# baggepinnen/LPVSpectral.jl

Hardware: AMD Instinct MI355X
Metric: signals/sec, ls_sparse_spectral_lpv group lasso N=2^20 Nf=512 Nv=8 (2000 ADMM iters; iters/sec in admm_iters_per_sec) (higher is better)
Workload: dtype f64

## Files before the change

lpvspectral.jl_amd/csrc/admm_one_launch.hip:

```cpp
#include "lpvs_internal.h"
#include "admm_device.h"
#include "admm_host.h"
#include "tile_order.h"

#include <algorithm>
#include <map>
#include <mutex>
#include <tuple>
#include <vector>
#include <cmath>
#include <cstdlib>
#include <string>
#include <type_traits>

namespace lpvs {

enum { FI_FIRST = 0, FI_MID = 1, FI_LAST = 2 };
typedef void (*FiKernel)(AdmmParams, const unsigned char *, const unsigned char *, int, int, long long, int, int, int, size_t, int);
static FiKernel fi_kernel(int mode, bool small, bool batch, bool nt, bool pa, bool f32);

__device__ __forceinline__ double wave_max(double v) {
#pragma unroll
    for (int o = 32; o > 0; o >>= 1) v = fmax(v, __shfl_xor(v, o, 64));
    return v;
// ... 41 lines not shown
    const int64_t r = (int64_t)blockIdx.x * 4 + wave;
    if (r >= n) return;
    const double2 *m2 = reinterpret_cast<const double2 *>(M + ((int64_t)blockIdx.y * np + r) * np);
    double acc = 0;
    for (int64_t j = lane; j < np / 2; j += 64) { const double2 m = m2[j]; acc += fabs(m.x) + fabs(m.y); }
    acc = wave_sum(acc);
    if (lane == 0) atomicMax(out + 2 * blockIdx.y, (unsigned long long)__double_as_longlong(acc));
}
__global__ void __launch_bounds__(256)
fi_state_kernel(AdmmParams p, int nblk, long long base, int with_consts) {
    const int sg = blockIdx.x, nprob = gridDim.x;
    const FiBufs f = fi_views(p.fi, (int64_t)nprob * p.np, nprob * nblk, nprob);
    const int64_t voff = (int64_t)sg * p.np;
    __shared__ double sh[3][4];
    double mx = 0, mr = 0, mu_ = 0;
    int bad = 0;
    for (int64_t e = threadIdx.x; e < p.np; e += 256) {
        const double a = p.xb[voff + e], b = p.rhs[voff + e], c = p.u[voff + e];
        mx = fmax(mx, fabs(a)); mr = fmax(mr, fabs(b)); mu_ = fmax(mu_, fabs(c));
        bad |= !(fabs(b) < 0x1p1000) || !(fabs(c) < 0x1p1000);
    }
    mx = wave_max(mx); mr = wave_max(mr); mu_ = wave_max(mu_);
    if ((threadIdx.x & 63) == 0) { sh[0][threadIdx.x >> 6] = mx; sh[1][threadIdx.x >> 6] = mr; sh[2][threadIdx.x >> 6] = mu_; }
    __syncthreads();
    mx = fmax(fmax(sh[0][0], sh[0][1]), fmax(sh[0][2], sh[0][3]));
    mr = fmax(fmax(sh[1][0], sh[1][1]), fmax(sh[1][2], sh[1][3]));
    mu_ = fmax(fmax(sh[2][0], sh[2][1]), fmax(sh[2][2], sh[2][3]));
    if (__syncthreads_or(bad)) { mr = __longlong_as_double(0x7ff0000000000000ll); mu_ = mr; }
    const int p1 = (int)((base + 1) & 1), p2 = (int)(base & 1);
    const int nbt = nprob * nblk, boff = sg * nblk;
    for (int b = threadIdx.x; b < nblk; b += 256) {
        f.rec[p1 * nbt + boff + b] = make_double2(mr, mu_);
        f.rec[p2 * nbt + boff + b] = make_double2(0.0, p.mu * mr);
        f.bn[boff + b] = 0.0; f.bn[nbt + boff + b] = 0.0;
    }
    if (threadIdx.x == 0) {
        if (with_consts) f.consts[2 * sg + 1] = mx;
        f.qbuf[sg] = 0.0; f.qbuf[nprob + sg] = 0.0;
    }
}

__device__ __forceinline__ void fi_fixed_product(const FixRaw &fr, const double *sI, const double *sJ, int wave, int lane, double (&v)[8], double (&tc)[8]) {
    const int c = lane & 15, gq = lane >> 4;
    double rj[8];
#pragma unroll
    for (int k = 0; k < 4; ++k) { rj[k] = sJ[4 * c + k]; rj[4 + k] = sJ[64 + 4 * c + k]; }
#pragma unroll
    for (int k = 0; k < 8; ++k) tc[k] = 0.0;
    const float stv[8] = {fr.st[0].x, fr.st[0].y, fr.st[0].z, fr.st[0].w, fr.st[1].x, fr.st[1].y, fr.st[1].z, fr.st[1].w};
    const unsigned int nw[8] = {fr.nq[0].x, fr.nq[0].y, fr.nq[0].z, fr.nq[0].w, fr.nq[1].x, fr.nq[1].y, fr.nq[1].z, fr.nq[1].w};
    double ri = (double)stv[0] * sI[wave * 32 + gq];
#pragma unroll
    for (int rg = 0; rg < 8; ++rg) {
        const double step = (double)stv[rg];
        const double ri_next = rg + 1 < 8 ? (double)stv[rg + 1] * sI[wave * 32 + 4 * (rg + 1) + gq] : 0.0;
        const int hh[8] = {fr.ha[rg].x, fr.ha[rg].y, fr.ha[rg].z, fr.ha[rg].w, fr.hb[rg].x, fr.hb[rg].y, fr.hb[rg].z, fr.hb[rg].w};
        double a0 = 0.0, a1 = 0.0;
#pragma unroll
        for (int k = 0; k < 8; k += 2) {
            const double m0 = fix_decode((unsigned int)hh[k], (nw[rg] >> (4 * k)) & 15u);
            const double m1 = fix_decode((unsigned int)hh[k + 1], (nw[rg] >> (4 * k + 4)) & 15u);
            tc[k] = opaque(fma(m0, ri, tc[k]));
            tc[k + 1] = opaque(fma(m1, ri, tc[k + 1]));
            a0 = fma(m0, rj[k], a0);
            a1 = fma(m1, rj[k + 1], a1);
        }
        v[rg] = step * (a0 + a1);
        ri = ri_next;
        __builtin_amdgcn_sched_barrier(0);
    }
}


#if defined(LPVS_TIMELINE) && LPVS_TIMELINE < 3
__device__ unsigned long long *g_lpvs_tl = nullptr;
extern "C" int32_t lpvs_debug_set_timeline(unsigned long long *dev_buf) {
    return hipMemcpyToSymbol(HIP_SYMBOL(g_lpvs_tl), &dev_buf, sizeof(dev_buf)) == hipSuccess ? LPVS_OK : LPVS_EDEVICE;
}
#define LPVS_TL_STAMP(k) do { if ((LPVS_TIMELINE >= 2 || (k) == 5) && tl_on && threadIdx.x == 0) tl_rec[k] = __builtin_amdgcn_s_memrealtime(); } while (0)
#else
#define LPVS_TL_STAMP(k) do { } while (0)
#endif

template <int MODE, int NK, bool BATCH, bool NT, bool PA, bool F32, bool NIBR = false>
__device__ __forceinline__ void
fi_one_tile_body(const AdmmParams &p, const unsigned char *__restrict__ Mp, const unsigned char *__restrict__ types, int ntiles, int nblk, long long g, int aslot,
                 int uslot , int commit_prev, size_t mp_stride) {
    constexpr bool prefetch_all = PA;
#if defined(LPVS_TIMELINE) && LPVS_TIMELINE < 3
    const bool tl_on = MODE == FI_MID && !BATCH && !F32 && g_lpvs_tl != nullptr;
    unsigned long long *tl_rec = tl_on ? g_lpvs_tl + ((size_t)(g & 1) * (size_t)ntiles + blockIdx.x) * 8 : nullptr;
    if (tl_on && threadIdx.x == 0) {
        tl_rec[0] = (unsigned long long)g; tl_rec[1] = __builtin_amdgcn_s_memrealtime();
        tl_rec[7] = __builtin_amdgcn_s_getreg((32 - 1) << 11 | 0 << 6 | 4);
    }
#endif
    __shared__ double sI[TS], sJ[TS], sT[4][TS], sq[2 * TS], red[3][4];
    const int sg = BATCH ? (int)blockIdx.y : 0, nprob = BATCH ? (int)gridDim.y : 1;
    const int64_t voff = (int64_t)sg * p.np;
    const int boff = sg * nblk, nbt = nprob * nblk;
    const FiBufs f = fi_views(p.fi, (int64_t)nprob * p.np, nbt, nprob);
    Mp += (size_t)sg * mp_stride; types += (size_t)sg * (size_t)ntiles;
    const int lane = threadIdx.x & 63, wave = threadIdx.x >> 6;
    const int bx = (MODE == FI_LAST || BATCH) ? (int)blockIdx.x : tile_order_index((int)blockIdx.x, nblk, p.tile_order & (int)(g & 1));
    int I, J;
    if (MODE == FI_LAST || bx < nblk) { I = J = bx; }
    else {
        const int k = bx - nblk;
        I = (int)((1.0 + sqrt(1.0 + 8.0 * (double)k)) * 0.5);
        while (I * (I - 1) / 2 > k) --I;
        while ((I + 1) * I / 2 <= k) ++I;
        J = k - I * (I - 1) / 2;
    }
    const int t = I * (I + 1) / 2 + J;
#if defined(LPVS_TIMELINE) && LPVS_TIMELINE < 3
    if (tl_on && threadIdx.x == 0) tl_rec[6] = __builtin_amdgcn_s_getreg((4 - 1) << 11 | 0 << 6 | 20) | (unsigned long long)t << 8;
#endif
    const unsigned char *tile = Mp + (size_t)t * (F32 ? (size_t)TS * TS * 4 : kSplitTileBytes);
    const unsigned char ttype = (MODE == FI_LAST || F32) ? 0 : types[t];
    AdmmStatus *status = p.status + sg;
    const int conv_flag = __builtin_nontemporal_load(&status->converged);
    const int blk = threadIdx.x < TS ? I : J, i = threadIdx.x & (TS - 1);
    const int64_t e = (int64_t)blk * TS + i;
    const bool ok = e < p.n;
    const int pg = (int)(g & 1), pg1 = pg ^ 1;
    double rhs_mem = 0, xbv = 0, uv = 0, qprev = 0;
    long long accp = 0;
    if (MODE == FI_FIRST) rhs_mem = p.rhs[voff + e];
    else {
        accp = f.acc((aslot + 2) % 3)[voff + e];
        xbv = p.xb[voff + e];
        uv = (uslot ? f.ualt : p.u)[voff + e];
        qprev = f.qbuf[pg1 * nprob + sg];
    }
    double bnv[NK];
    double2 recv[NK];
#pragma unroll
    for (int k = 0; k < NK; ++k) {
        const int b = lane + 64 * k < nblk ? lane + 64 * k : nblk - 1;
        bnv[k] = MODE != FI_FIRST ? f.bn[pg * nbt + boff + b] : 0.0;
        recv[k] = MODE != FI_LAST ? f.rec[pg * nbt + boff + b] : make_double2(0.0, 0.0);
    }
    const double Rrow = BATCH ? f.consts[2 * sg] : p.fi_R, xbmax = BATCH ? f.consts[2 * sg + 1] : p.fi_xbmax;
    __builtin_amdgcn_sched_barrier(0);
    FixRaw fr;
    float4 fha[8], fhb[8];
    double diag_pre = 0.0;
    if (MODE != FI_LAST && F32) {
        typedef unsigned int u32x4b __attribute__((ext_vector_type(4)));
        const __amdgpu_buffer_rsrc_t rs = __builtin_amdgcn_make_buffer_rsrc(const_cast<unsigned char *>(tile), 0, TS * TS * 4, 0x00020000);
        const int off_head = ((wave * 32 + (lane >> 4)) * TS + 4 * (lane & 15)) * 4;
#pragma unroll
        for (int rg = 0; rg < 8; ++rg) {
            fha[rg] = __builtin_bit_cast(float4, (u32x4b)__builtin_amdgcn_raw_buffer_load_b128(rs, off_head, rg * (4 * TS * 4), 0));
            fhb[rg] = __builtin_bit_cast(float4, (u32x4b)__builtin_amdgcn_raw_buffer_load_b128(rs, off_head, rg * (4 * TS * 4) + 256, 0));
        }
    }
    if (MODE != FI_LAST && !F32) {
        typedef unsigned int u32x4b __attribute__((ext_vector_type(4)));
        constexpr int aux = NT ? 2 : 0;
        const int tbytes = I != J ? (int)kMixedFixedTileBytes : (prefetch_all ? (int)kMixedFixedTileBytes + TS * 8 : 0);
        const __amdgpu_buffer_rsrc_t rs = __builtin_amdgcn_make_buffer_rsrc(const_cast<unsigned char *>(tile), 0, tbytes, 0x00020000);
        const __amdgpu_buffer_rsrc_t rs_nq = __builtin_amdgcn_make_buffer_rsrc(const_cast<unsigned char *>(tile), 0, p.mp_fix32 ? 0 : tbytes, 0x00020000);
        const int gq_ = lane >> 4, c_ = lane & 15;
        const int off_head = ((wave * 32 + gq_) * TS + 4 * c_) * 4;
        const int off_nq = (int)kFixHeadBytes + (wave * 64 + lane) * 32, off_st = (int)(kFixHeadBytes + kFixNibBytes) + (wave * 4 + gq_) * 32;
        fr.nq[0] = __builtin_bit_cast(uint4, (u32x4b)__builtin_amdgcn_raw_buffer_load_b128(rs_nq, off_nq, 0, aux));
        fr.nq[1] = __builtin_bit_cast(uint4, (u32x4b)__builtin_amdgcn_raw_buffer_load_b128(rs_nq, off_nq, 16, aux));
        fr.st[0] = __builtin_bit_cast(float4, (u32x4b)__builtin_amdgcn_raw_buffer_load_b128(rs, off_st, 0, aux));
        fr.st[1] = __builtin_bit_cast(float4, (u32x4b)__builtin_amdgcn_raw_buffer_load_b128(rs, off_st, 16, aux));
#pragma unroll
        for (int rg = 0; rg < 8; ++rg) {
            fr.ha[rg] = __builtin_bit_cast(int4, (u32x4b)__builtin_amdgcn_raw_buffer_load_b128(rs, off_head, rg * (4 * TS * 4), aux));
            fr.hb[rg] = __builtin_bit_cast(int4, (u32x4b)__builtin_amdgcn_raw_buffer_load_b128(rs, off_head, rg * (4 * TS * 4) + 256, aux));
        }
        if (PA) {
            const int rgo = ((c_ & 8) ? 4 : 0) + ((c_ & 4) ? 2 : 0) + ((c_ & 2) ? 1 : 0);
            typedef unsigned int u32x2b __attribute__((ext_vector_type(2)));
            const u32x2b dw = __builtin_amdgcn_raw_buffer_load_b64(rs, (int)(kFixHeadBytes + kFixNibBytes) + TS * 4 + (wave * 32 + 4 * rgo + gq_) * 8, 0, 0);
            diag_pre = __builtin_bit_cast(double, dw);
        }
    }
    __builtin_amdgcn_sched_barrier(0);
    double mR = 0, mU = 0;
#pragma unroll
    for (int k = 0; k < NK; ++k) { mR = fmax(mR, recv[k].x); mU = fmax(mU, recv[k].y); }
    if (conv_flag) return;
    if (MODE != FI_FIRST && commit_prev && (p.tol > 0.0 || blockIdx.x == 0)) {
        double part = 0.0;
#pragma unroll
        for (int k = 0; k < NK; ++k) part += lane + 64 * k < nblk ? bnv[k] : 0.0;
        const double nxz = sqrt(wave_sum(part));
        const bool conv = nxz < p.tol;
        if (blockIdx.x == 0 && threadIdx.x == 0) commit_iteration(status, nxz, p.tol);
        if (conv) return;
    }
    double rhs_v;
    if (MODE == FI_FIRST) rhs_v = rhs_mem;
    else {
        const double xi = ok ? xbv + (double)accp * qprev : 0.0;
        const double ui = ok ? uv : 0.0;
        const double v = xi + ui;
        double zi = 0.0;
        if (p.prox_kind == LPVS_PROX_L1) {
            zi = prox_l1(v, p.mu * p.prox_param);
        } else if (p.prox_kind == LPVS_PROX_L0) {
            zi = prox_l0(v, sqrt(2.0 * p.mu * p.prox_param));
        } else {
            const int gl = (int)p.group_len;
            sq[threadIdx.x] = v * v;
            __syncthreads();
            const double *grp = sq + (threadIdx.x & TS) + (i / gl) * gl;
            double s2 = 0;
            for (int q = 0; q < gl; ++q) s2 += grp[q];
            zi = group_scale(s2, p.prox_param * p.mu) * v;
        }
        if (!ok) zi = 0.0;
        const DualStep t = dual_step(xi, ui, zi, 0.0, p.mu, ok, true);
        const double d = t.d, un = t.un;
        rhs_v = t.rhs;
        if (I == J) {
            const bool own = threadIdx.x < TS;
            if (own) {
                p.x[voff + e] = xi; p.z[voff + e] = zi;
                (MODE == FI_LAST ? p.u : (uslot ? p.u : f.ualt))[voff + e] = un;
                if (MODE == FI_LAST) p.rhs[voff + e] = rhs_v;
            }
            const double d2 = own && ok ? d * d : 0.0;
            const double inf_ = __longlong_as_double(0x7ff0000000000000ll);
            const double ar = fabs(rhs_v) < inf_ ? fabs(rhs_v) : inf_, au = fabs(un) < inf_ ? fabs(un) : inf_;
            const double w0 = wave_sum(d2), w1 = wave_max(own ? ar : 0.0), w2 = wave_max(own ? au : 0.0);
            if (lane == 0) { red[0][wave] = w0; red[1][wave] = w1; red[2][wave] = w2; }
            __syncthreads();
            if (threadIdx.x == 0) {
                f.bn[pg1 * nbt + boff + I] = red[0][0] + red[0][1];
                f.rec[pg1 * nbt + boff + I] = make_double2(fmax(red[1][0], red[1][1]), fmax(red[2][0], red[2][1]));
            }
        }
    }
    if (MODE == FI_LAST) return;
    LPVS_TL_STAMP(2);
    if (I == J && threadIdx.x < TS) f.acc((aslot + 1) % 3)[voff + e] = 0;
    if (threadIdx.x < TS) sI[i] = rhs_v; else sJ[i] = rhs_v;
    mR = wave_max_nonneg(mR); mU = wave_max_nonneg(mU);
    double B = Rrow * ((xbmax + Rrow * mR + mU) / p.mu) * 1.000001;
    const bool bound_ok = B < 0x1p1000;
    if (!(B > 0x1p-900)) B = 0x1p-900;
    int eb = 0;
    (void)frexp(bound_ok ? B : 1.0, &eb);
    const double quantum = bound_ok ? ldexp(1.0, eb - 62) : __longlong_as_double(0x7ff8000000000000ll), invq = bound_ok ? ldexp(1.0, 62 - eb) : 0.0;
    if (blockIdx.x == 0 && threadIdx.x == 0) f.qbuf[pg * nprob + sg] = quantum;
    __syncthreads();
    LPVS_TL_STAMP(3);
    const int c = lane & 15, gq = lane >> 4;
    double rj[8], tc[8], v[8];
    const double *diag = nullptr;
    if (F32) {
#pragma unroll
        for (int k = 0; k < 4; ++k) { rj[k] = sJ[4 * c + k]; rj[4 + k] = sJ[64 + 4 * c + k]; }
#pragma unroll
        for (int k = 0; k < 8; ++k) tc[k] = 0.0;
#pragma unroll
        for (int rg = 0; rg < 8; ++rg) {
            const double ri = sI[wave * 32 + 4 * rg + gq];
            const float hh[8] = {fha[rg].x, fha[rg].y, fha[rg].z, fha[rg].w, fhb[rg].x, fhb[rg].y, fhb[rg].z, fhb[rg].w};
            double a0 = 0.0, a1 = 0.0;
#pragma unroll
            for (int k = 0; k < 8; k += 2) {
                const double m0 = (double)hh[k], m1 = (double)hh[k + 1];
                tc[k] = opaque(fma(m0, ri, tc[k]));
                tc[k + 1] = opaque(fma(m1, ri, tc[k + 1]));
                a0 = fma(m0, rj[k], a0);
                a1 = fma(m1, rj[k + 1], a1);
            }
            v[rg] = a0 + a1;
            __builtin_amdgcn_sched_barrier(0);
        }
    } else if (PA || ttype != 0) {
        if (!PA && I == J) {
            FixRaw fd;
            fix_load(tile, wave, lane, fd, p.mp_fix32 != 0 ? 1 : 0);
            fi_fixed_product(fd, sI, sJ, wave, lane, v, tc);
        } else fi_fixed_product(fr, sI, sJ, wave, lane, v, tc);
        if (ttype == 2 && !prefetch_all) diag = reinterpret_cast<const double *>(tile + kFixHeadBytes + kFixNibBytes + TS * 4);
    } else {
#pragma unroll
        for (int k = 0; k < 4; ++k) { rj[k] = sJ[4 * c + k]; rj[4 + k] = sJ[64 + 4 * c + k]; }
#pragma unroll
        for (int k = 0; k < 8; ++k) tc[k] = 0.0;
        const float *head = reinterpret_cast<const float *>(tile) + (wave * 32 + gq) * TS + 4 * c;
        const unsigned short *tail = reinterpret_cast<const unsigned short *>(tile + (size_t)TS * TS * 4) + (wave * 32 + gq) * TS + 8 * c;
#pragma unroll
        for (int half = 0; half < 2; ++half) {
            float4 ha[4], hb[4];
            uint4 lq[4];
#pragma unroll
            for (int r4 = 0; r4 < 4; ++r4) {
                const int rg = 4 * half + r4;
                ha[r4] = load16<NT, float4>(head + rg * 4 * TS);
                hb[r4] = load16<NT, float4>(head + rg * 4 * TS + 64);
                lq[r4] = load16<NT, uint4>(tail + rg * 4 * TS);
            }
#pragma unroll
            for (int r4 = 0; r4 < 4; ++r4) {
                const int rg = 4 * half + r4;
                const double ri = sI[wave * 32 + 4 * rg + gq];
                const float hh[8] = {ha[r4].x, ha[r4].y, ha[r4].z, ha[r4].w, hb[r4].x, hb[r4].y, hb[r4].z, hb[r4].w};
                const unsigned int qq[8] = {lq[r4].x & 0xffffu, lq[r4].x >> 16, lq[r4].y & 0xffffu, lq[r4].y >> 16,
                                            lq[r4].z & 0xffffu, lq[r4].z >> 16, lq[r4].w & 0xffffu, lq[r4].w >> 16};
                double a0 = 0.0, a1 = 0.0;
#pragma unroll
                for (int k = 0; k < 8; k += 2) {
                    const double m0 = split_decode(hh[k], qq[k]), m1 = split_decode(hh[k + 1], qq[k + 1]);
                    tc[k] = opaque(fma(m0, ri, tc[k]));
                    tc[k + 1] = opaque(fma(m1, ri, tc[k + 1]));
                    a0 = fma(m0, rj[k], a0);
                    a1 = fma(m1, rj[k + 1], a1);
                }
                v[rg] = a0 + a1;
            }
        }
    }
    LPVS_TL_STAMP(4);
#pragma unroll
    for (int m = 8, cnt = 4; m >= 2; m >>= 1, cnt >>= 1) {
        const bool up = (c & m) != 0;
#pragma unroll
        for (int k = 0; k < cnt; ++k) {
            const double lo_ = opaque(v[k]), hi_ = opaque(v[k + cnt]);
            v[k] = (up ? hi_ : lo_) + __shfl_xor(up ? lo_ : hi_, m, 64);
        }
    }
    v[0] += __shfl_xor(v[0], 1, 64);
    unsigned long long *acc_cur = reinterpret_cast<unsigned long long *>(f.acc(aslot));
    if ((c & 1) == 0) {
        const int rg = ((c & 8) ? 4 : 0) + ((c & 4) ? 2 : 0) + ((c & 2) ? 1 : 0);
        const int row = wave * 32 + 4 * rg + gq;
        const double r1 = diag != nullptr ? fma(diag[row], sI[row], v[0]) : (PA && I == J ? fma(diag_pre, sI[row], v[0]) : v[0]);
        atomicAdd(acc_cur + voff + (int64_t)I * TS + row, (unsigned long long)__double2ll_rn(r1 * invq));
    }
    if (I != J) {
#pragma unroll
        for (int m = 32, cnt = 4; m >= 16; m >>= 1, cnt >>= 1) {
            const bool up = (lane & m) != 0;
#pragma unroll
            for (int k = 0; k < cnt; ++k) {
                const double lo_ = opaque(tc[k]), hi_ = opaque(tc[k + cnt]);
                tc[k] = (up ? hi_ : lo_) + __shfl_xor(up ? lo_ : hi_, m, 64);
            }
        }
        const int col = ((lane & 32) ? 64 : 0) + 4 * c + ((lane & 16) ? 2 : 0);
        sT[wave][col] = tc[0]; sT[wave][col + 1] = tc[1];
        __syncthreads();
        if (threadIdx.x < TS) {
            const double r2 = ((sT[0][threadIdx.x] + sT[1][threadIdx.x]) + sT[2][threadIdx.x]) + sT[3][threadIdx.x];
            atomicAdd(acc_cur + voff + (int64_t)J * TS + threadIdx.x, (unsigned long long)__double2ll_rn(r2 * invq));
        }
    }
    if constexpr (NIBR && !F32) {
        if (ttype != 0) {
            __syncthreads();
            FixRaw fb;
            fix_load(tile, wave, lane, fb, 2);
            double vn[8], tn[8];
            fi_fixed_product(fb, sI, sJ, wave, lane, vn, tn);
            unsigned long long *acc_n = reinterpret_cast<unsigned long long *>(p.nib_acc);
#pragma unroll
            for (int m = 8, cnt = 4; m >= 2; m >>= 1, cnt >>= 1) {
                const bool up = (c & m) != 0;
#pragma unroll
                for (int k = 0; k < cnt; ++k) {
                    const double lo_ = opaque(vn[k]), hi_ = opaque(vn[k + cnt]);
                    vn[k] = (up ? hi_ : lo_) + __shfl_xor(up ? lo_ : hi_, m, 64);
                }
            }
            vn[0] += __shfl_xor(vn[0], 1, 64);
            if ((c & 1) == 0) {
                const int rg = ((c & 8) ? 4 : 0) + ((c & 4) ? 2 : 0) + ((c & 2) ? 1 : 0);
                atomicAdd(acc_n + voff + (int64_t)I * TS + wave * 32 + 4 * rg + gq, (unsigned long long)__double2ll_rn(vn[0] * invq));
            }
            if (I != J) {
#pragma unroll
                for (int m = 32, cnt = 4; m >= 16; m >>= 1, cnt >>= 1) {
                    const bool up = (lane & m) != 0;
#pragma unroll
                    for (int k = 0; k < cnt; ++k) {
                        const double lo_ = opaque(tn[k]), hi_ = opaque(tn[k + cnt]);
                        tn[k] = (up ? hi_ : lo_) + __shfl_xor(up ? lo_ : hi_, m, 64);
                    }
                }
                const int col = ((lane & 32) ? 64 : 0) + 4 * c + ((lane & 16) ? 2 : 0);
                sT[wave][col] = tn[0]; sT[wave][col + 1] = tn[1];
                __syncthreads();
                if (threadIdx.x < TS) {
                    const double r2 = ((sT[0][threadIdx.x] + sT[1][threadIdx.x]) + sT[2][threadIdx.x]) + sT[3][threadIdx.x];
                    atomicAdd(acc_n + voff + (int64_t)J * TS + threadIdx.x, (unsigned long long)__double2ll_rn(r2 * invq));
                }
            }
        }
    }
    LPVS_TL_STAMP(5);
}

template <int MODE, int NK, bool BATCH, bool NT, bool PA, bool F32, bool NIBR = false>
__global__ void __launch_bounds__(256, 3)
admm_iter_mixed_kernel(AdmmParams p, const unsigned char *__restrict__ Mp, const unsigned char *__restrict__ types, int ntiles, int nblk, long long g, int aslot,
                       int uslot, int commit_prev, size_t mp_stride, int ) {
    fi_one_tile_body<MODE, NK, BATCH, NT, PA, F32, NIBR>(p, Mp, types, ntiles, nblk, g, aslot, uslot, commit_prev, mp_stride);
}
__global__ void __launch_bounds__(256)
nib_acc_commit_kernel(long long *__restrict__ acc, const double *__restrict__ quantum, const double *__restrict__ xb_corr, double *__restrict__ xb, int64_t np) {
    const int64_t i = (int64_t)blockIdx.x * 256 + threadIdx.x;
    if (i >= np) return;
    const int64_t e = (int64_t)blockIdx.y * np + i;
    xb[e] = xb_corr[e] + (double)acc[e] * quantum[blockIdx.y];
    acc[e] = 0;
}

__global__ void set_double_kernel(double *dst, double v) { *dst = v; }
int32_t launch_fi_setup(const AdmmParams &p, long long base, bool with_consts, hipStream_t s, double r_known) {
    const int nblk = (int)(p.np / TS), nprob = p.ns;
    const FiBufs f = fi_views(p.fi, (int64_t)nprob * p.np, nprob * nblk, nprob);
    if (with_consts) {
        LPVS_HIP(hipMemsetAsync(f.consts, 0, sizeof(double) * 2 * (size_t)nprob, s));
        if (r_known > 0 && nprob == 1) hipLaunchKernelGGL(set_double_kernel, dim3(1), dim3(1), 0, s, f.consts, r_known);
        else hipLaunchKernelGGL(fi_rowsum_kernel, dim3((unsigned)ceil_div(p.np, 4), (unsigned)nprob), dim3(256), 0, s, p.M, p.np, p.n, reinterpret_cast<unsigned long long *>(f.consts));
    }
    hipLaunchKernelGGL(fi_state_kernel, dim3((unsigned)nprob), dim3(256), 0, s, p, nblk, base, with_consts ? 1 : 0);
    LPVS_HIP(hipGetLastError());
    return LPVS_OK;
}

__global__ void __launch_bounds__(256)
fi_fixup_kernel(AdmmParams p, int nblk, long long base, long long iters) {
    const int sg = blockIdx.y, nprob = gridDim.y;
    const AdmmStatus *status = p.status + sg;
    if (!status->converged) return;
    const long long ic = status->iters - base - 1;
    if (ic < 0 || ic > iters - 2 || ((ic + 1) & 1) == 0) return;
    const FiBufs f = fi_views(p.fi, (int64_t)nprob * p.np, nprob * nblk, nprob);
    const int64_t e = (int64_t)blockIdx.x * 256 + threadIdx.x;
    if (e < p.np) p.u[(int64_t)sg * p.np + e] = f.ualt[(int64_t)sg * p.np + e];
}
__global__ void __launch_bounds__(64)
fi_commit_kernel(AdmmParams p, int nblk, int par) {
    const int sg = blockIdx.x, nprob = gridDim.x;
    AdmmStatus *status = p.status + sg;
    if (status->converged) return;
    const FiBufs f = fi_views(p.fi, (int64_t)nprob * p.np, nprob * nblk, nprob);
    __shared__ double slot;
    const double nxz = pending_norm(f.bn + (int64_t)par * nprob * nblk + (int64_t)sg * nblk, nblk, &slot);
    if (threadIdx.x == 0) commit_iteration(status, nxz, p.tol);
}

int32_t fi_read_consts(const AdmmParams &p, double out[2], hipStream_t s) {
    const FiBufs f = fi_views(p.fi, p.np, (int)(p.np / TS));
    LPVS_HIP(hipMemcpyAsync(out, f.consts, sizeof(double) * 2, hipMemcpyDeviceToHost, s));
    LPVS_HIP(hipStreamSynchronize(s));
    return LPVS_OK;
}

template <int NK, bool BATCH, bool NT, bool PA, bool F32 = false>
static FiKernel fi_kernel_mode(int mode) {
    return mode == FI_FIRST ? admm_iter_mixed_kernel<FI_FIRST, NK, BATCH, NT, PA, F32> : mode == FI_MID ? admm_iter_mixed_kernel<FI_MID, NK, BATCH, NT, PA, F32>
                                                                                                       : admm_iter_mixed_kernel<FI_LAST, NK, BATCH, NT, PA, F32>;
}
static FiKernel fi_kernel(int mode, bool small, bool batch, bool nt, bool pa, bool f32 = false) {
    if (f32) return small ? fi_kernel_mode<1, false, false, true, true>(mode) : fi_kernel_mode<6, false, false, true, true>(mode);
    if (batch) {
        if (nt) return pa ? fi_kernel_mode<1, true, true, true>(mode) : fi_kernel_mode<1, true, true, false>(mode);
        return pa ? fi_kernel_mode<1, true, false, true>(mode) : fi_kernel_mode<1, true, false, false>(mode);
    }
    if (small) return pa ? fi_kernel_mode<1, false, false, true>(mode) : fi_kernel_mode<1, false, false, false>(mode);
    if (nt) return pa ? fi_kernel_mode<6, false, true, true>(mode) : fi_kernel_mode<6, false, true, false>(mode);
    return pa ? fi_kernel_mode<6, false, false, true>(mode) : fi_kernel_mode<6, false, false, false>(mode);
}
bool nib_fused_applies(const AdmmParams &p) {
    const char *e = experiment_env("LPVS_NIB_FUSED");
    return !(e && e[0] == '0') && p.nib_period > 0 && p.nib_acc != nullptr && p.mp_types != nullptr && p.fi_prefetch_all == 0 && fi_applicable(p);
}
template <bool NT, bool PA> static FiKernel fi_kernel_nibr_batch(int mode) {
    return mode == FI_FIRST ? admm_iter_mixed_kernel<FI_FIRST, 1, true, NT, PA, false, true> : admm_iter_mixed_kernel<FI_MID, 1, true, NT, PA, false, true>;
}
static FiKernel fi_kernel_nibr(int mode, bool small, bool nt, bool batch = false, bool pa = false) {
    if (batch) { if (nt) return pa ? fi_kernel_nibr_batch<true, true>(mode) : fi_kernel_nibr_batch<true, false>(mode);
                 return pa ? fi_kernel_nibr_batch<false, true>(mode) : fi_kernel_nibr_batch<false, false>(mode); }
    if (small) return mode == FI_FIRST ? admm_iter_mixed_kernel<FI_FIRST, 1, false, false, false, false, true> : admm_iter_mixed_kernel<FI_MID, 1, false, false, false, false, true>;
    if (nt) return mode == FI_FIRST ? admm_iter_mixed_kernel<FI_FIRST, 6, false, true, false, false, true> : admm_iter_mixed_kernel<FI_MID, 6, false, true, false, false, true>;
    return mode == FI_FIRST ? admm_iter_mixed_kernel<FI_FIRST, 6, false, false, false, false, true> : admm_iter_mixed_kernel<FI_MID, 6, false, false, false, false, true>;
}
int32_t launch_fi_chunk(const AdmmParams &p, int64_t iters, bool batch, size_t mp_stride, bool prefetch_all, hipStream_t s) {
    const int nblk = (int)(p.np / TS), nprob = batch ? p.ns : 1;
    const unsigned ntiles = (unsigned)(nblk * (nblk + 1) / 2);
    const FiBufs f = fi_views(p.fi, (int64_t)nprob * p.np, nprob * nblk, nprob);
    const unsigned char *Mp = reinterpret_cast<const unsigned char *>(p.Mp);
    LPVS_HIP(hipMemsetAsync(f.acc(0), 0, sizeof(long long) * (size_t)p.np * (size_t)nprob, s));
    const long long base = p.fi_base;
    const bool small = nblk <= 64;
    const int nto = option_in_effect(LPVS_OPT_NT_LOADS, p.opt_nt_loads);
    const size_t stream_bytes = batch ? (size_t)ntiles * kSplitTileBytes * (size_t)nprob : (size_t)ntiles * kMixedFixedTileBytes;
    const bool nt = (batch || !small) && !p.mp_f32 && (nto ? nto == LPVS_NT_ON : stream_bytes > ((size_t)240 << 20));
    auto launch = [&](int mode, unsigned grid, long long g, int aslot, int uslot, int commit_prev) {
        hipLaunchKernelGGL(fi_kernel(mode, small, batch, nt, prefetch_all, p.mp_f32 != 0), dim3(grid, (unsigned)nprob), dim3(256), 0, s, p, Mp, p.mp_types, (int)ntiles, nblk, g, aslot, uslot,
                           commit_prev, mp_stride, prefetch_all ? 1 : 0);
    };
    const bool nib = batch ? (p.nib_period > 0 && p.nib_acc != nullptr && p.xb_corr != nullptr && p.mp_types != nullptr) : (!prefetch_all && nib_fused_applies(p));
    auto refresh_due = [&](long long g) { return p.nib_period > 0 && nib_refresh_due(g, p.nib_period, p.nib_ramp); };
    auto launch_step = [&](int mode, long long g, int aslot, int uslot, int commit_prev, const double *u_after) -> int32_t {
        const bool due = refresh_due(g);
        if (due && nib) {
            hipLaunchKernelGGL(fi_kernel_nibr(mode, small, nt, batch, prefetch_all), dim3(ntiles, (unsigned)nprob), dim3(256), 0, s, p, Mp, p.mp_types, (int)ntiles, nblk, g, aslot, uslot, commit_prev,
                               mp_stride, prefetch_all ? 1 : 0);
            hipLaunchKernelGGL(nib_acc_commit_kernel, dim3((unsigned)ceil_div(p.np, 256), (unsigned)nprob), dim3(256), 0, s, p.nib_acc, (const double *)(f.qbuf + (g & 1) * nprob), p.xb_corr,
                               const_cast<double *>(p.xb), p.np);
            return LPVS_OK;
        }
        launch(mode, ntiles, g, aslot, uslot, commit_prev);
        if (due && !batch) return launch_nibble_refresh(p, u_after != nullptr, u_after, s);
        return LPVS_OK;
    };
    LPVS_TRY(launch_step(FI_FIRST, base, 0, 0, 0, nullptr));
    for (int64_t j = 1; j < iters; ++j)
        LPVS_TRY(launch_step(FI_MID, base + j, (int)(j % 3), (int)((j - 1) & 1), j >= 2 ? 1 : 0, ((j - 1) & 1) ? p.u : f.ualt));
    launch(FI_LAST, (unsigned)nblk, base + iters, (int)(iters % 3), (int)((iters - 1) & 1), iters >= 2 ? 1 : 0);
    hipLaunchKernelGGL(fi_fixup_kernel, dim3((unsigned)ceil_div(p.np, 256), (unsigned)nprob), dim3(256), 0, s, p, nblk, base, (long long)iters);
    hipLaunchKernelGGL(fi_commit_kernel, dim3((unsigned)nprob), dim3(64), 0, s, p, nblk, (int)((base + iters - 1) & 1));
    LPVS_HIP(hipGetLastError());
    return LPVS_OK;
}

}
```

lpvspectral.jl_amd/csrc/api.hip:

```cpp
#include <cmath>
#include <cstdarg>
#include <cstdio>
#include <cstdlib>
#include <cstring>
#include <ctime>
#include <map>
#include <mutex>
#include <array>
#include <thread>
#include <string>
#include <vector>

#include "lpvs_internal.h"

namespace lpvs {

static thread_local char g_err[512] = "";

void set_error(const char *fmt, ...) {
    va_list ap;
    va_start(ap, fmt);
    vsnprintf(g_err, sizeof(g_err), fmt, ap);
    va_end(ap);
}
// ... 493 lines not shown
    }
    h->M_valid = true; h->M_shift = shift;
    return LPVS_OK;
}


StoragePlan decide_plan(lpvs_problem *h) {
    const int xc_opt = option_in_effect(LPVS_OPT_XUPDATE_CORRECTION, h->opt[LPVS_OPT_XUPDATE_CORRECTION]);
    const bool corrected = h->np >= kSymmetricMinNp && xc_opt != LPVS_XCORR_OFF;
    h->xcorr = xcorr_schedule_from(corrected ? experiment_env("LPVS_XUPDATE_CORRECTION") : nullptr, xcorr_default_schedule(h->ns, corrected));
    const int storage = option_in_effect(LPVS_OPT_M_STORAGE, h->opt[LPVS_OPT_M_STORAGE]);
    return admm_storage_plan(h->np, h->ns, h->f32, storage, h->ns > 1 && multi_signal_fixed_tiles_ok(h->np), h->xcorr.on(), fix_bits_from(experiment_env),
                             nib_knobs_from(experiment_env));
}

int32_t pack_mixed(lpvs_problem *h, const StoragePlan &want, StoragePlan *stored) {
    hipStream_t s = h->stream;
    const PackedLayout lay = packed_layout(h->np, want.element_bytes, 1);
    unsigned char *types = mp_tile_types(h->Mp, h->np, 1);
    unsigned long long *amax = reinterpret_cast<unsigned long long *>(h->Mp.as<unsigned char>() + lay.absmax_off);
    LPVS_TRY(launch_pack_tiles_mixed(h->M.as<double>(), h->np, h->Mp.as<unsigned char>(), types, amax, s, want.diag_float,
                                     want.want_rowsum ? h->part.as<double>() : nullptr, h->n, want.want_rowsum ? h->scratch.as<double>() : nullptr, want.fix_bits));
    std::vector<unsigned char> ht(lay.tiles);
    unsigned long long rbits = 0;
    LPVS_HIP(hipMemcpyAsync(ht.data(), types, lay.tiles, hipMemcpyDeviceToHost, s));
    if (want.want_rowsum) LPVS_HIP(hipMemcpyAsync(&rbits, amax + 1, sizeof(rbits), hipMemcpyDeviceToHost, s));
    LPVS_HIP(hipStreamSynchronize(s));
    if (want.want_rowsum) memcpy(&h->Mp_rowsum, &rbits, sizeof(double));
    h->Mp_census = tile_census(ht.data(), lay.tiles);
    if (getenv("LPVS_TRACE")) fprintf(stderr, "[lpvs] mixed packing: %zu of %zu tiles fixed point (%zu diagonal), ns = %lld\n", h->Mp_census.fixed, lay.tiles, (size_t)(h->np / kTile), (long long)h->ns);
    if (demote_to_split(h->Mp_census.fixed, lay.tiles)) {
        LPVS_TRY(launch_pack_tiles_split(h->M.as<double>(), h->np, h->Mp.as<unsigned char>(), s));
        h->Mp_census = TileCensus{};
        h->Mp_demoted = true;
        *stored = demoted_plan(want);
    }
    return LPVS_OK;
}

int32_t pack_inverse(lpvs_problem *h, const StoragePlan &want) {
    hipStream_t s = h->stream;
    h->Mp_demoted = false;
    if (!h->Mp.p || h->Mp.bytes < want.bytes) LPVS_TRY(h->Mp.alloc(want.bytes));
    h->Mp_census = TileCensus{};
    StoragePlan stored = want;
    if (want.mode == kMpF32) LPVS_TRY(launch_pack_tiles_f32(h->M.as<double>(), h->np, h->Mp.as<float>(), s));
    else if (want.mode == kMpSplit) LPVS_TRY(launch_pack_tiles_split(h->M.as<double>(), h->np, h->Mp.as<unsigned char>(), s));
    else if (want.mode == kMpMixed) LPVS_TRY(pack_mixed(h, want, &stored));
    else LPVS_TRY(launch_pack_tiles(h->M.as<double>(), h->np, h->Mp.as<double>(), s));
    h->plan = stored; h->Mp_valid = true;
    return LPVS_OK;
}

int32_t start_state(lpvs_problem *h, const double *x0) {
    hipStream_t s = h->stream;
    LPVS_HIP(hipMemsetAsync(h->part.p, 0, h->part.bytes, s));
    const size_t v = sizeof(double) * (size_t)h->np * (size_t)h->ns;
    LPVS_HIP(hipMemsetAsync(h->x.p, 0, v, s));
    if (x0) LPVS_TRY(copy_state_in(h, h->x.p, x0));
    std::vector<double> hb((size_t)h->np * (size_t)h->ns, 0.0);
    LPVS_HIP(hipMemcpyAsync(hb.data(), h->b.p, v, hipMemcpyDeviceToHost, s));
    LPVS_HIP(hipStreamSynchronize(s));
    if (h->sign < 0) for (auto &q : hb) q = -q;
    return copy_to_device(h->bs.p, hb.data(), v, s);
}

int32_t offset_vectors(lpvs_problem *h) {
    hipStream_t s = h->stream;
    const size_t v = sizeof(double) * (size_t)h->np * (size_t)h->ns;
    if (!h->xb.p) LPVS_TRY(h->xb.alloc(v));
    int steps = 1;
    if (const char *e = experiment_env("LPVS_XB_REFINE")) steps = atoi(e) < 0 ? 0 : atoi(e);
    h->xb_refined = steps > 0;
    LPVS_TRY(launch_offset_vector_refined(h->G.as<double>(), h->M.as<double>(), h->np, h->n, (int)h->ns, h->bs.as<double>(), h->M_shift, steps,
                                          h->xb.as<double>(), h->rhs.as<double>(), h->scratch.as<double>(), s));
    if (h->xcorr.on()) {
        if (!h->xb0.p) LPVS_TRY(h->xb0.alloc(v));
        if (!h->corr.p) LPVS_TRY(h->corr.alloc(3 * v));
        LPVS_HIP(hipMemcpyAsync(h->xb0.p, h->xb.p, v, hipMemcpyDeviceToDevice, s));
    }
    if (h->plan.nib_period > 0) {
        if (!h->xb_corr.p) LPVS_TRY(h->xb_corr.alloc(v));
        if (!h->nib_rhs.p) LPVS_TRY(h->nib_rhs.alloc(v));
        if (!h->nib_acc.p) LPVS_TRY(h->nib_acc.alloc(v));
        LPVS_HIP(hipMemsetAsync(h->nib_acc.p, 0, v, s));
        if (!h->nib_part.p) LPVS_TRY(h->nib_part.alloc(sizeof(double) * 2 * packed_tiles(h->np) * 128));
        LPVS_HIP(hipMemcpyAsync(h->xb_corr.p, h->xb.p, v, hipMemcpyDeviceToDevice, s));
    }
    return LPVS_OK;
}

int32_t one_launch_constants(lpvs_problem *h, const AdmmParams &p) {
    hipStream_t s = h->stream;
    if (h->Mp_rowsum > 0 && h->plan.mode == kMpMixed) {
        AdmmParams pr = p; pr.fi_R = h->Mp_rowsum;
        LPVS_TRY(launch_fi_setup(pr, 0, true, s, h->Mp_rowsum));
    } else LPVS_TRY(launch_fi_setup(p, 0, true, s));
    double hc[2] = {0, 0};
    LPVS_TRY(fi_read_consts(p, hc, s));
    h->fi_R = hc[0]; h->fi_xbmax = hc[1] * (1.0 + 0x1p-20); h->fi_sync = 0;
    return LPVS_OK;
}

int32_t restore_initial_offset(lpvs_problem *h) {
    hipStream_t s = h->stream;
    const size_t v = sizeof(double) * (size_t)h->np * (size_t)h->ns;
    LPVS_HIP(hipMemcpyAsync(h->xb.p, h->xb0.p, v, hipMemcpyDeviceToDevice, s));
    if (h->plan.nib_period > 0 && h->xb_corr.p) {
        LPVS_HIP(hipMemcpyAsync(h->xb_corr.p, h->xb0.p, v, hipMemcpyDeviceToDevice, s));
        LPVS_HIP(hipMemsetAsync(h->nib_acc.p, 0, v, s));
    }
    return LPVS_OK;
}

int32_t correct_offset(lpvs_problem *h, const AdmmParams &p) {
    LPVS_TRY(launch_xupdate_correction(p, h->G.as<double>(), h->M_shift, h->xb_refined ? nullptr : h->bs.as<double>(), h->xb0.as<double>(), h->xb.as<double>(),
                                       h->corr.as<double>(), h->stream));
    if (p.nib_period > 0) LPVS_TRY(launch_nibble_refresh(p, false, nullptr, h->stream, true));
    return LPVS_OK;
}
int32_t timed_correction(lpvs_problem *h, const AdmmParams &p, size_t i) {
    if (h->xc_ev.size() < 2 * (i + 1)) {
        hipEvent_t ea = nullptr, eb = nullptr;
        LPVS_HIP(hipEventCreate(&ea)); h->xc_ev.push_back(ea);
        LPVS_HIP(hipEventCreate(&eb)); h->xc_ev.push_back(eb);
    }
    LPVS_HIP(hipEventRecord(h->xc_ev[2 * i], h->stream));
    LPVS_TRY(correct_offset(h, p));
    LPVS_HIP(hipEventRecord(h->xc_ev[2 * i + 1], h->stream));
    return LPVS_OK;
}

int32_t read_status(lpvs_problem *h, std::vector<AdmmStatus> &st, bool *all_converged) {
    LPVS_HIP(hipMemcpyAsync(st.data(), h->status.p, sizeof(AdmmStatus) * st.size(), hipMemcpyDeviceToHost, h->stream));
    LPVS_HIP(hipStreamSynchronize(h->stream));
    *all_converged = true;
    for (auto &q : st) *all_converged = *all_converged && q.converged;
    return LPVS_OK;
}

int32_t capture_graph(lpvs_problem *h, const AdmmParams &p, int64_t chunk) {
    hipStream_t s = h->stream;
    hipGraph_t g = nullptr;
    LPVS_HIP(hipStreamBeginCapture(s, hipStreamCaptureModeThreadLocal));
    const int32_t rc = launch_admm_iterations(p, chunk, s);
    const hipError_t e = hipStreamEndCapture(s, &g);
    if (rc != LPVS_OK || e != hipSuccess || g == nullptr) {
        (void)hipGetLastError();
        if (g) (void)hipGraphDestroy(g);
        set_error("hipGraph capture of the ADMM chunk failed");
        return LPVS_EDEVICE;
    }
    const hipError_t ei = hipGraphInstantiate(&h->admm_graph, g, nullptr, nullptr, 0);
    (void)hipGraphDestroy(g);
    if (ei != hipSuccess) { (void)hipGetLastError(); h->admm_graph = nullptr; set_error("hipGraphInstantiate failed"); return LPVS_EDEVICE; }
    h->admm_graph_iters = chunk;
    return LPVS_OK;
}

int32_t enqueue_run(lpvs_problem *h, AdmmParams &p, IterationKind kind, int64_t max_iters, std::vector<AdmmStatus> &st, size_t *nxc) {
    hipStream_t s = h->stream;
    if (kind == IterationKind::one_launch && h->fi_sync != p.fi_base) LPVS_TRY(launch_fi_setup(p, p.fi_base, false, s));
    LPVS_HIP(hipEventRecord(h->ev[0].a, s));
    int64_t todo = max_iters;
    const int64_t chunk = graph_chunk_iters(kind);
    if (h->admm_graph && h->admm_graph_iters != chunk) h->drop_graph();
    const int64_t replays = graph_replays(h->np, todo, chunk, h->np < kSymmetricMinNp && getenv("LPVS_NO_GRAPH") == nullptr);
    if (replays > 0 && !h->admm_graph) LPVS_TRY(capture_graph(h, p, chunk));
    for (int64_t i = 0; i < replays; ++i) { LPVS_HIP(hipGraphLaunch(h->admm_graph, s)); todo -= chunk; }
    while (todo > 0) {
        const RunStep r = next_run_step(h->xcorr, h->k_enq, todo);
        LPVS_TRY(launch_admm_iterations(p, r.step, s));
        h->n_nib += (double)nib_refreshes_between(p.fi_base, p.fi_base + r.step, p.nib_period, p.nib_ramp);
        todo -= r.step; h->k_enq += r.step;
        if (!r.correct_after) continue;
        LPVS_TRY(timed_correction(h, p, (*nxc)++));
        if (todo > 0 && !(h->tol > 0)) p.fi_base += r.step;
        else if (todo > 0) {
            bool all = false;
            LPVS_TRY(read_status(h, st, &all));
            if (all) break;
            p.fi_base = st[0].iters;
        }
    }
    LPVS_HIP(hipEventRecord(h->ev[0].b, s));
    return LPVS_OK;
}

void fold_timings(lpvs_problem *h, size_t nxc, long long iters_before, long long iters_after) {
    for (size_t i = 0; i < nxc; ++i) {
        float ms = 0;
        if (hipEventElapsedTime(&ms, h->xc_ev[2 * i], h->xc_ev[2 * i + 1]) == hipSuccess) { h->t_xcorr += ms; h->n_xcorr += 1; } else (void)hipGetLastError();
    }
    h->t_admm += h->ev[0].ms(); h->admm_iters_timed += (double)(iters_after - iters_before);
}

}

struct PanelBufs { DevBuf P, Wp, slab, scr; const double *Wdev = nullptr; int64_t ld = 0; };

template <class Fill>
static int32_t panel_tables(lpvs_problem *h, const GramPlan &pl, const double *W, int64_t N, PanelBufs &t, Fill fill) {
    hipStream_t s = h->stream;
    const int64_t Npad = pl.ksplit * pl.rows_per_chunk, ld = t.ld = round_up(h->n, 256);
    LPVS_TRY(t.P.alloc(sizeof(double) * (size_t)Npad * (size_t)ld));
    if (Npad > N) LPVS_HIP(hipMemsetAsync(t.P.as<double>() + N * ld, 0, sizeof(double) * (size_t)(Npad - N) * (size_t)ld, s));
    if (W != nullptr) {
        LPVS_TRY(t.Wp.alloc(sizeof(double) * (size_t)Npad));
        LPVS_HIP(hipMemsetAsync(t.Wp.p, 0, t.Wp.bytes, s));
        LPVS_TRY(copy_to_device(t.Wp.p, W, sizeof(double) * (size_t)N, s));
        t.Wdev = t.Wp.as<double>();
    }
    LPVS_HIP(hipEventRecord(h->ev[0].a, s));
    LPVS_TRY(fill(t.P.as<double>(), ld));
    LPVS_HIP(hipEventRecord(h->ev[0].b, s));
    return LPVS_OK;
}

template <class Fill>
static int32_t create_panel_problem(lpvs_problem *h, const double *y, const double *W, int64_t N, Fill fill) {
    hipStream_t s = h->stream;
    const GramPlan pl = make_gram_plan(h->n, N);
    DevArg dy;
    LPVS_TRY(dy.set(y, N, s));
    LPVS_TRY(open_problem(h, 1, ZeroGram::all));
    PanelBufs t;
    DrainOnExit drain(s);
    LPVS_TRY(panel_tables(h, pl, W, N, t, fill));
    LPVS_TRY(t.slab.alloc(pl.slab_bytes));
    LPVS_TRY(t.scr.alloc(rhs_scratch_bytes(N, h->n)));
    LPVS_HIP(hipEventRecord(h->ev[1].a, s));
    LPVS_TRY(launch_gram_panel(pl, t.P.as<double>(), t.ld, t.Wdev, t.slab.as<double>(), s, &h->gram_stage));
    LPVS_HIP(hipEventRecord(h->ev[1].b, s));
    LPVS_HIP(hipEventRecord(h->ev[2].a, s));
    LPVS_TRY(launch_gram_reduce(pl, t.slab.as<double>(), h->G.as<double>(), h->np, s));
    LPVS_TRY(launch_rhs_panel(t.P.as<double>(), t.ld, h->n, t.Wdev, dy.p, N, h->b.as<double>(), t.scr.as<double>(), t.scr.bytes, s));
    LPVS_HIP(hipEventRecord(h->ev[2].b, s));
    return close_problem(h, GramForm::panel, dense_issued_flops(pl), pl.ksplit);
}

static int32_t fourier_slots(const double *f, int64_t Nf, const double *t_dev, int64_t N, double *tam, hipStream_t s, ApSlots &sl) {
    std::vector<double> hw;
    LPVS_TRY(fetch_host(hw, f, Nf));
    for (auto &v : hw) v = 6.283185307179586 * v;
    double tlo, thi;
// ... 2423 lines not shown
```

Measured before the change: 15.44.

## Fold nibble-accumulator commit into the next ADMM iteration kernel via triple buffering

For single problems, the pending nibble-refresh commit (xb += nib_acc * quantum, then zero the accumulator) now happens inside the following iteration kernel instead of in a separate commit step. The nib_acc buffer is tripled and rotated through a control word, so the refresh that is writing, the commit that is reading and the clearing each use a different slot. This is meant to remove an extra kernel launch and a full-vector pass per refresh. The cost is three times the accumulator memory, extra kernel template variants, and an added memset whenever the fi setup is rerun.

```diff
diff --git a/lpvspectral.jl_amd/csrc/admm_one_launch.hip b/lpvspectral.jl_amd/csrc/admm_one_launch.hip
--- a/lpvspectral.jl_amd/csrc/admm_one_launch.hip
+++ b/lpvspectral.jl_amd/csrc/admm_one_launch.hip
@@ -147,10 +147,11 @@
 #define LPVS_TL_STAMP(k) do { } while (0)
 #endif
 
-template <int MODE, int NK, bool BATCH, bool NT, bool PA, bool F32, bool NIBR = false>
+template <int MODE, int NK, bool BATCH, bool NT, bool PA, bool F32, bool NIBR = false, bool PEND = false>
 __device__ __forceinline__ void
 fi_one_tile_body(const AdmmParams &p, const unsigned char *__restrict__ Mp, const unsigned char *__restrict__ types, int ntiles, int nblk, long long g, int aslot,
-                 int uslot , int commit_prev, size_t mp_stride) {
+                 int uslot , int commit_prev, size_t mp_stride, int nibctl) {
+    static_assert(!PEND || (!BATCH && !F32 && MODE != FI_FIRST), "a pending commit: single problems, in the launch that updates");
     constexpr bool prefetch_all = PA;
 #if defined(LPVS_TIMELINE) && LPVS_TIMELINE < 3
     const bool tl_on = MODE == FI_MID && !BATCH && !F32 && g_lpvs_tl != nullptr;
@@ -194,9 +195,12 @@
     if (MODE == FI_FIRST) rhs_mem = p.rhs[voff + e];
     else {
         accp = f.acc((aslot + 2) % 3)[voff + e];
-        xbv = p.xb[voff + e];
+        long long nibp = 0;
+        if constexpr (PEND) { xbv = p.xb_corr[voff + e]; nibp = p.nib_acc[(int64_t)((nibctl >> 2) & 3) * p.np + e]; }
+        else xbv = p.xb[voff + e];
         uv = (uslot ? f.ualt : p.u)[voff + e];
         qprev = f.qbuf[pg1 * nprob + sg];
+        if constexpr (PEND) xbv = __dadd_rn(xbv, __dmul_rn((double)nibp, qprev));
     }
     double bnv[NK];
     double2 recv[NK];
@@ -290,6 +294,10 @@
                 p.x[voff + e] = xi; p.z[voff + e] = zi;
                 (MODE == FI_LAST ? p.u : (uslot ? p.u : f.ualt))[voff + e] = un;
                 if (MODE == FI_LAST) p.rhs[voff + e] = rhs_v;
+                if constexpr (PEND) {
+                    const_cast<double *>(p.xb)[voff + e] = xbv;
+                    p.nib_acc[(int64_t)((nibctl >> 4) & 3) * p.np + e] = 0;
+                }
             }
             const double d2 = own && ok ? d * d : 0.0;
             const double inf_ = __longlong_as_double(0x7ff0000000000000ll);
@@ -429,7 +437,7 @@
             fix_load(tile, wave, lane, fb, 2);
             double vn[8], tn[8];
             fi_fixed_product(fb, sI, sJ, wave, lane, vn, tn);
-            unsigned long long *acc_n = reinterpret_cast<unsigned long long *>(p.nib_acc);
+            unsigned long long *acc_n = reinterpret_cast<unsigned long long *>(p.nib_acc) + (BATCH ? (int64_t)0 : (int64_t)(nibctl & 3) * p.np);
 #pragma unroll
             for (int m = 8, cnt = 4; m >= 2; m >>= 1, cnt >>= 1) {
                 const bool up = (c & m) != 0;
@@ -467,11 +475,11 @@
     LPVS_TL_STAMP(5);
 }
 
-template <int MODE, int NK, bool BATCH, bool NT, bool PA, bool F32, bool NIBR = false>
+template <int MODE, int NK, bool BATCH, bool NT, bool PA, bool F32, bool NIBR = false, bool PEND = false>
 __global__ void __launch_bounds__(256, 3)
 admm_iter_mixed_kernel(AdmmParams p, const unsigned char *__restrict__ Mp, const unsigned char *__restrict__ types, int ntiles, int nblk, long long g, int aslot,
-                       int uslot, int commit_prev, size_t mp_stride, int ) {
-    fi_one_tile_body<MODE, NK, BATCH, NT, PA, F32, NIBR>(p, Mp, types, ntiles, nblk, g, aslot, uslot, commit_prev, mp_stride);
+                       int uslot, int commit_prev, size_t mp_stride, int nibctl ) {
+    fi_one_tile_body<MODE, NK, BATCH, NT, PA, F32, NIBR, PEND>(p, Mp, types, ntiles, nblk, g, aslot, uslot, commit_prev, mp_stride, nibctl);
 }
 __global__ void __launch_bounds__(256)
 nib_acc_commit_kernel(long long *__restrict__ acc, const double *__restrict__ quantum, const double *__restrict__ xb_corr, double *__restrict__ xb, int64_t np) {
@@ -553,6 +561,14 @@
     if (small) return mode == FI_FIRST ? admm_iter_mixed_kernel<FI_FIRST, 1, false, false, false, false, true> : admm_iter_mixed_kernel<FI_MID, 1, false, false, false, false, true>;
     if (nt) return mode == FI_FIRST ? admm_iter_mixed_kernel<FI_FIRST, 6, false, true, false, false, true> : admm_iter_mixed_kernel<FI_MID, 6, false, true, false, false, true>;
     return mode == FI_FIRST ? admm_iter_mixed_kernel<FI_FIRST, 6, false, false, false, false, true> : admm_iter_mixed_kernel<FI_MID, 6, false, false, false, false, true>;
+}
+template <int NK, bool NT> static FiKernel fi_kernel_pend_nk(int mode, bool nibr) {
+    if (mode == FI_LAST) return admm_iter_mixed_kernel<FI_LAST, NK, false, NT, false, false, false, true>;
+    return nibr ? admm_iter_mixed_kernel<FI_MID, NK, false, NT, false, false, true, true> : admm_iter_mixed_kernel<FI_MID, NK, false, NT, false, false, false, true>;
+}
+static FiKernel fi_kernel_pend(int mode, bool small, bool nt, bool nibr) {
+    if (small) return fi_kernel_pend_nk<1, false>(mode, nibr);
+    return nt ? fi_kernel_pend_nk<6, true>(mode, nibr) : fi_kernel_pend_nk<6, false>(mode, nibr);
 }
 int32_t launch_fi_chunk(const AdmmParams &p, int64_t iters, bool batch, size_t mp_stride, bool prefetch_all, hipStream_t s) {
     const int nblk = (int)(p.np / TS), nprob = batch ? p.ns : 1;
@@ -571,8 +587,19 @@
     };
     const bool nib = batch ? (p.nib_period > 0 && p.nib_acc != nullptr && p.xb_corr != nullptr && p.mp_types != nullptr) : (!prefetch_all && nib_fused_applies(p));
     auto refresh_due = [&](long long g) { return p.nib_period > 0 && nib_refresh_due(g, p.nib_period, p.nib_ramp); };
+    const bool nib_single = nib && !batch;
+    auto pending = [&](long long g) { return nib_single && g > base && refresh_due(g - 1); };
+    auto nib_ctl = [&](long long g) {
+        const long long r = nib_refreshes_between(0, g, p.nib_period, p.nib_ramp);
+        return (int)(r % 3) | (int)((r + 2) % 3) << 2 | (int)((r + 1) % 3) << 4;
+    };
     auto launch_step = [&](int mode, long long g, int aslot, int uslot, int commit_prev, const double *u_after) -> int32_t {
         const bool due = refresh_due(g);
+        if (nib_single && (due || pending(g))) {
+            const FiKernel k = pending(g) ? fi_kernel_pend(mode, small, nt, due) : fi_kernel_nibr(mode, small, nt);
+            hipLaunchKernelGGL(k, dim3(ntiles, 1u), dim3(256), 0, s, p, Mp, p.mp_types, (int)ntiles, nblk, g, aslot, uslot, commit_prev, mp_stride, nib_ctl(g));
+            return LPVS_OK;
+        }
         if (due && nib) {
             hipLaunchKernelGGL(fi_kernel_nibr(mode, small, nt, batch, prefetch_all), dim3(ntiles, (unsigned)nprob), dim3(256), 0, s, p, Mp, p.mp_types, (int)ntiles, nblk, g, aslot, uslot, commit_prev,
                                mp_stride, prefetch_all ? 1 : 0);
@@ -587,7 +614,10 @@
     LPVS_TRY(launch_step(FI_FIRST, base, 0, 0, 0, nullptr));
     for (int64_t j = 1; j < iters; ++j)
         LPVS_TRY(launch_step(FI_MID, base + j, (int)(j % 3), (int)((j - 1) & 1), j >= 2 ? 1 : 0, ((j - 1) & 1) ? p.u : f.ualt));
-    launch(FI_LAST, (unsigned)nblk, base + iters, (int)(iters % 3), (int)((iters - 1) & 1), iters >= 2 ? 1 : 0);
+    if (pending(base + iters))
+        hipLaunchKernelGGL(fi_kernel_pend(FI_LAST, small, nt, false), dim3((unsigned)nblk, 1u), dim3(256), 0, s, p, Mp, p.mp_types, (int)ntiles, nblk, base + iters, (int)(iters % 3),
+                           (int)((iters - 1) & 1), iters >= 2 ? 1 : 0, mp_stride, nib_ctl(base + iters));
+    else launch(FI_LAST, (unsigned)nblk, base + iters, (int)(iters % 3), (int)((iters - 1) & 1), iters >= 2 ? 1 : 0);
     hipLaunchKernelGGL(fi_fixup_kernel, dim3((unsigned)ceil_div(p.np, 256), (unsigned)nprob), dim3(256), 0, s, p, nblk, base, (long long)iters);
     hipLaunchKernelGGL(fi_commit_kernel, dim3((unsigned)nprob), dim3(64), 0, s, p, nblk, (int)((base + iters - 1) & 1));
     LPVS_HIP(hipGetLastError());
diff --git a/lpvspectral.jl_amd/csrc/api.hip b/lpvspectral.jl_amd/csrc/api.hip
--- a/lpvspectral.jl_amd/csrc/api.hip
+++ b/lpvspectral.jl_amd/csrc/api.hip
@@ -599,8 +599,8 @@
     if (h->plan.nib_period > 0) {
         if (!h->xb_corr.p) LPVS_TRY(h->xb_corr.alloc(v));
         if (!h->nib_rhs.p) LPVS_TRY(h->nib_rhs.alloc(v));
-        if (!h->nib_acc.p) LPVS_TRY(h->nib_acc.alloc(v));
-        LPVS_HIP(hipMemsetAsync(h->nib_acc.p, 0, v, s));
+        if (!h->nib_acc.p) LPVS_TRY(h->nib_acc.alloc(3 * v));
+        LPVS_HIP(hipMemsetAsync(h->nib_acc.p, 0, 3 * v, s));
         if (!h->nib_part.p) LPVS_TRY(h->nib_part.alloc(sizeof(double) * 2 * packed_tiles(h->np) * 128));
         LPVS_HIP(hipMemcpyAsync(h->xb_corr.p, h->xb.p, v, hipMemcpyDeviceToDevice, s));
     }
@@ -625,7 +625,7 @@
     LPVS_HIP(hipMemcpyAsync(h->xb.p, h->xb0.p, v, hipMemcpyDeviceToDevice, s));
     if (h->plan.nib_period > 0 && h->xb_corr.p) {
         LPVS_HIP(hipMemcpyAsync(h->xb_corr.p, h->xb0.p, v, hipMemcpyDeviceToDevice, s));
-        LPVS_HIP(hipMemsetAsync(h->nib_acc.p, 0, v, s));
+        LPVS_HIP(hipMemsetAsync(h->nib_acc.p, 0, 3 * v, s));
     }
     return LPVS_OK;
 }
@@ -677,7 +677,10 @@
 
 int32_t enqueue_run(lpvs_problem *h, AdmmParams &p, IterationKind kind, int64_t max_iters, std::vector<AdmmStatus> &st, size_t *nxc) {
     hipStream_t s = h->stream;
-    if (kind == IterationKind::one_launch && h->fi_sync != p.fi_base) LPVS_TRY(launch_fi_setup(p, p.fi_base, false, s));
+    if (kind == IterationKind::one_launch && h->fi_sync != p.fi_base) {
+        LPVS_TRY(launch_fi_setup(p, p.fi_base, false, s));
+        if (h->plan.nib_period > 0 && h->nib_acc.p) LPVS_HIP(hipMemsetAsync(h->nib_acc.p, 0, 3 * sizeof(double) * (size_t)h->np * (size_t)h->ns, s));
+    }
     LPVS_HIP(hipEventRecord(h->ev[0].a, s));
     int64_t todo = max_iters;
     const int64_t chunk = graph_chunk_iters(kind);
```

After: 15.44. No clear change (-0.0%).
